# kaylode/vehicle-counting

Measured on AMD Instinct MI355X. Metric: end-to-end frames/sec (detect+NMS+ReID+track), YOLOv5s 640px, higher is better.
Workload: dtype bf16; 1 GPU; YOLOv5s 640x640 single camera stream per GPU, bf16 convs (BASELINE.json configs[1]); workload_id=s640-bf16, clip_frames=512, objects=12, num_classes=80, detection_injection=False, weights=seeded synthetic (no checkpoints available), streams=1, ranks=1, counts_allgather_via=vc_allgather_counts (RCCL, C ABI), tracked_rows=155352, tracker=device-resident (one kernel per batch, no host round trip per frame)

## Files before the change

### vehicle-counting_amd/csrc/conv_cfgs.h

```cpp
#pragma once

namespace vc {

#define VC_CONV_CFGS(X)                                                                                          \
    X(0, 256, 32, 4, 1, 4, 2)   X(1, 128, 64, 2, 2, 4, 2)   X(2, 128, 128, 2, 2, 4, 2)  X(3, 64, 64, 2, 2, 4, 2)      \
    X(4, 128, 64, 2, 2, 8, 2)   X(5, 128, 128, 2, 2, 8, 2)  X(6, 64, 64, 2, 2, 8, 2)    X(7, 256, 64, 4, 1, 4, 2)     \
    X(8, 256, 64, 4, 1, 8, 2)   X(9, 256, 128, 2, 2, 4, 2)  X(10, 256, 128, 2, 2, 8, 2) X(11, 64, 128, 1, 4, 4, 2)    \
    X(12, 64, 128, 1, 4, 8, 2)  X(13, 256, 32, 4, 1, 8, 2)                                                          \
    X(14, 64, 64, 2, 2, 4, 4)   X(15, 64, 64, 2, 2, 8, 3)   X(16, 64, 64, 2, 2, 8, 4)   X(17, 128, 64, 2, 2, 4, 4)    \
    X(18, 128, 64, 2, 2, 8, 3)  X(19, 128, 128, 2, 2, 4, 4) X(20, 128, 128, 2, 2, 8, 3) X(21, 64, 128, 1, 4, 4, 4)    \
    X(22, 64, 128, 1, 4, 8, 3)  X(23, 256, 32, 4, 1, 4, 4)  X(24, 256, 64, 4, 1, 4, 4)  X(25, 256, 64, 4, 1, 8, 3)    \
    X(26, 256, 128, 2, 2, 4, 4) X(27, 256, 128, 2, 2, 8, 3)
#define VC_HALO_CFGS(Y) Y(28, 128, 64, 2, 2, 2) Y(29, 128, 64, 2, 2, 3) Y(30, 128, 128, 2, 2, 2) Y(31, 128, 128, 2, 2, 3) \
                        Y(36, 128, 64, 4, 1, 2) Y(37, 128, 64, 4, 1, 3) Y(38, 256, 128, 4, 1, 2) Y(39, 256, 128, 4, 1, 3)
#define VC_CONV_BIG_CFGS(X) X(40, 256, 256, 4, 4, 4, 2) X(41, 256, 256, 4, 4, 4, 3) X(42, 256, 256, 4, 4, 4, 4) X(43, 256, 256, 4, 4, 8, 2)
#define VC_S2HALO_CFGS(V) V(44, 128, 128, 2, 2, 2) V(45, 128, 128, 2, 2, 3) V(46, 256, 128, 4, 1, 3) V(47, 128, 128, 2, 2, 4) \
                          V(48, 128, 256, 2, 2, 2) V(49, 256, 128, 4, 1, 2)
#define VC_DIRECT_CFGS(Z) Z(32, 2, 1, 4, 4) Z(33, 4, 2, 4, 2) Z(34, 4, 2, 2, 3) Z(35, 4, 4, 2, 2)
#define VC_STREAM_CFGS(S) S(50, 8, 4, 4, 2) S(51, 16, 8, 2, 2) S(52, 8, 8, 2, 1) S(53, 16, 4, 2, 2) S(54, 8, 4, 2, 1)
#define VC_HALO_V2_CFGS(W) W(55)
#define VC_CONV_DEEP_CFGS(X) X(60, 64, 64, 2, 2, 8, 6) X(61, 64, 64, 2, 2, 8, 8) X(62, 128, 64, 2, 2, 8, 6) X(63, 64, 128, 1, 4, 8, 6)
#define VC_SK_CFGS(K) K(56, 64, 64, 2, 2, 8, 3) K(57, 64, 64, 2, 2, 8, 4) K(58, 128, 64, 2, 2, 8, 3) K(59, 64, 128, 1, 4, 8, 3)
#define VC_PAIR_CFGS(P) P(64, 256, 128, 4, 2, 4, 3) P(65, 128, 256, 2, 4, 4, 3) P(66, 256, 128, 4, 2, 4, 2)
#define VC_PAIR4_CFGS(P) P(67, 256, 128, 2, 2, 4, 3) P(68, 256, 128, 2, 2, 4, 2)
#define VC_DIRECT8_CFGS(F) F(69, 4, 1, 2, 2) F(70, 4, 2, 2, 2) F(71, 4, 1, 4, 2) F(72, 8, 1, 2, 2)

enum ConvFamily : int { FAM_IGEMM, FAM_HALO, FAM_HALO_V2, FAM_HALO_S2, FAM_DIRECT, FAM_STREAM, FAM_DIRECT8 };
struct ConvCfgEntry { int id; ConvFamily family; };
#define VC_REG_IGEMM(i, ...) {i, FAM_IGEMM},
#define VC_REG_HALO(i, ...) {i, FAM_HALO},
#define VC_REG_HALO_V2(i, ...) {i, FAM_HALO_V2},
#define VC_REG_HALO_S2(i, ...) {i, FAM_HALO_S2},
#define VC_REG_DIRECT(i, ...) {i, FAM_DIRECT},
#define VC_REG_STREAM(i, ...) {i, FAM_STREAM},
#define VC_REG_DIRECT8(i, ...) {i, FAM_DIRECT8},
constexpr ConvCfgEntry kConvCfgs[] = {
    VC_CONV_CFGS(VC_REG_IGEMM) VC_HALO_CFGS(VC_REG_HALO) VC_DIRECT_CFGS(VC_REG_DIRECT) VC_CONV_BIG_CFGS(VC_REG_IGEMM) VC_S2HALO_CFGS(VC_REG_HALO_S2)
    VC_STREAM_CFGS(VC_REG_STREAM) VC_HALO_V2_CFGS(VC_REG_HALO_V2) VC_SK_CFGS(VC_REG_IGEMM) VC_CONV_DEEP_CFGS(VC_REG_IGEMM) VC_PAIR_CFGS(VC_REG_IGEMM)
    VC_PAIR4_CFGS(VC_REG_IGEMM) VC_DIRECT8_CFGS(VC_REG_DIRECT8)};
#undef VC_REG_IGEMM
#undef VC_REG_HALO
#undef VC_REG_HALO_V2
#undef VC_REG_HALO_S2
#undef VC_REG_DIRECT
#undef VC_REG_STREAM
#undef VC_REG_DIRECT8
constexpr int kNumConvCfgs = (int)(sizeof(kConvCfgs) / sizeof(kConvCfgs[0]));

struct ConvFamilyTable { ConvFamily of[kNumConvCfgs]; bool ok; };
constexpr ConvFamilyTable conv_family_table() {
    ConvFamilyTable t{};
    int seen[kNumConvCfgs] = {};
    t.ok = true;
    for (const ConvCfgEntry& e : kConvCfgs) {
        if (e.id < 0 || e.id >= kNumConvCfgs || seen[e.id]++) { t.ok = false; continue; }
        t.of[e.id] = e.family;
    }
    return t;
}
constexpr ConvFamilyTable kConvFamily = conv_family_table();
static_assert(kConvFamily.ok, "tile configuration ids must be exactly 0 .. N - 1, each once");

#define VC_ID_HALO_V2(i) i
constexpr int kCfgHaloV2 = VC_HALO_V2_CFGS(VC_ID_HALO_V2);
#undef VC_ID_HALO_V2

}
```

### vehicle-counting_amd/csrc/conv_dispatch.hip

```cpp
#include <algorithm>
#include <cstdlib>

#include "vc_common.h"
#include "conv_cfgs.h"

namespace vc {

int conv_num_cfgs() { return kNumConvCfgs; }

bool conv_stream_cfg(int cfg) { return cfg >= 0 && cfg < kNumConvCfgs && kConvFamily.of[cfg] == FAM_STREAM; }

int conv_k_tile(int prec) { return prec == PREC_F32 ? 32 : prec == PREC_FP8 ? 128 : 64; }

double conv_flops(const ConvP& p) { return 2.0 * (double)p.M * (double)p.Cout * (double)p.K; }

static int conv_heuristic(const ConvP& p) {
    if (p.prec == PREC_FP8) {
        if (p.Cout <= 64) return 4;
        const long t = (long)((p.M + 127) / 128) * ((p.Cout + 127) / 128);
        return t >= 512 ? 5 : 6;
    }
    if (p.in_up) return 2;
    if (p.Cout <= 32) return 0;
    if (p.Cout <= 64) return 1;
    const long t128 = (long)((p.M + 127) / 128) * ((p.Cout + 127) / 128);
    return t128 >= 512 ? 2 : 3;
}

int launch_conv_cfg(const ConvP& p, int cfg, hipStream_t s) {
    if (cfg < 0 || cfg >= conv_num_cfgs()) cfg = conv_heuristic(p);
    switch (kConvFamily.of[cfg]) {
        case FAM_IGEMM: return launch_igemm_cfg(p, cfg, s);
        case FAM_HALO: return launch_halo_cfg(p, cfg, s);
        case FAM_HALO_V2: return launch_halo_v2_cfg(p, cfg, s);
        case FAM_HALO_S2: return launch_halo_s2_cfg(p, cfg, s);
        case FAM_DIRECT:
        case FAM_STREAM:
        case FAM_DIRECT8: return launch_pointwise_cfg(p, cfg, s);
    }
    return VC_ERR_ARG;
}

int conv_check(const ConvP& p);

int launch_conv(const ConvP& p, hipStream_t s) {
    VC_TRY(conv_check(p));
    const int rc = launch_conv_cfg(p, p.cfg, s);
    if (rc == VC_ERR_ARG && p.cfg >= 0 && p.cfg < conv_num_cfgs() && !getenv("VC_CONV_STRICT")) return launch_conv_cfg(p, -1, s);
    return rc;
}

int conv_check(const ConvP& p) {
    const int ch = p.prec == PREC_F32 ? 4 : p.prec == PREC_FP8 ? 16 : 8;
    if (p.prec == PREC_FP8)
        VC_CHECK(p.scale && p.Cout % 8 == 0 && p.out_cs % 8 == 0 && p.out_co % 8 == 0 && (p.split == 0 || (p.split % 8 == 0 && p.out2_cs % 8 == 0 && p.out2_co % 8 == 0)) &&
                 (p.res_mode == RES_NONE || (p.res_cs % 4 == 0 && p.res_co % 4 == 0)), VC_ERR_ARG, "conv fp8: channel scales / 8-channel alignment of the outputs");
    VC_CHECK(p.Cin % ch == 0 && p.in_cs % ch == 0 && p.in_co % ch == 0, VC_ERR_ARG,
             "conv: input channels/stride/offset (%d,%d,%d) must be multiples of %d", p.Cin, p.in_cs, p.in_co, ch);
    VC_CHECK(p.out_cs % 4 == 0 && p.out_co % 4 == 0, VC_ERR_ARG, "conv: output stride/offset must be multiples of 4");
    VC_CHECK(p.split == 0 || (p.split % 4 == 0 && p.out2 && p.out2_cs % 4 == 0 && p.out2_co % 4 == 0 && p.res_mode == RES_NONE), VC_ERR_ARG,
             "conv: bad split destination");
    VC_CHECK(!(p.prec == PREC_FP8 && p.out_bf16 && p.split != 0), VC_ERR_ARG, "conv fp8: the bf16 store has one destination (conv_epilogue_fp8 would put channels >= split behind the first slice)");
    VC_CHECK(p.res_mode == RES_NONE || (p.res_cs % 4 == 0 && p.res_co % 4 == 0), VC_ERR_ARG, "conv: residual alignment");
    VC_CHECK(p.Kp % conv_k_tile(p.prec) == 0 && p.Kp >= p.K, VC_ERR_ARG, "conv: bad K padding %d/%d", p.K, p.Kp);
    VC_CHECK(p.M > 0 && p.Cout > 0, VC_ERR_ARG, "conv: empty problem");
    VC_CHECK(!p.in_up || (p.prec == PREC_BF16 && p.kh == 1 && p.kw == 1 && p.sh == 1 && p.sw == 1 && p.ph == 0 && p.pw == 0 && p.H % 2 == 0 && p.W % 2 == 0 &&
                          p.up_C > 0 && p.up_C < p.Cin && p.up_C % 64 == 0 && p.Cin % 64 == 0 && p.up_cs % 8 == 0 && p.up_co % 8 == 0 && !p.m_dev), VC_ERR_ARG,
             "conv: the upsample fold-in needs a bf16 pointwise conv on an even-sized map with 64-channel-aligned halves");
    VC_CHECK((size_t)p.B * p.H * p.W * p.in_cs * elem_size(p.prec) < (1ull << 31), VC_ERR_CAPACITY, "conv: input tensor exceeds the 2 GiB buffer descriptor");
    VC_CHECK((size_t)((p.Cout + 127) / 128 * 128) * p.Kp * elem_size(p.prec) < (1ull << 31), VC_ERR_CAPACITY, "conv: weights exceed 2 GiB");
    VC_CHECK(p.kh * p.kw <= 40, VC_ERR_ARG, "conv: at most 40 taps (validity mask is 64 bits incl. K padding)");
    VC_CHECK(p.M < (1 << 24), VC_ERR_CAPACITY, "conv: more than 2^24 output pixels in one launch");
    VC_CHECK((size_t)p.M * std::max(p.out_cs, std::max(p.res_cs, p.out2_cs)) * ((p.prec == PREC_F32 || p.out_f32) ? 4 : (p.prec == PREC_FP8 && !p.out_bf16) ? 1 : 2) < (1ull << 31),
             VC_ERR_CAPACITY, "conv: output tensor exceeds 2 GiB (32-bit buffer offsets)");
    return VC_OK;
}

}
```

### vehicle-counting_amd/csrc/conv_launch.h

```cpp
#pragma once
#include <algorithm>
#include <cstdint>
#include <cstdio>
#include <cstdlib>
#include <vector>

#include "vc_common.h"
#include "conv_geom.h"

namespace vc {

struct ConvSwitches {
    bool sk;
    bool s2halo;
    bool direct;
    bool direct8;
    bool halo_v2;
    bool persist;
    bool balanced;
    bool sk_uncached;
    bool s2pw_store;
    int dyn_lds;
    int reserve;
};
inline const ConvSwitches& conv_switches() {
    static const ConvSwitches sw = [] {
        const auto num = [](const char* name, int dflt) { const char* v = getenv(name); return v ? atoi(v) : dflt; };
        ConvSwitches c;
        c.sk = num("VC_CONV_SK", 1) != 0;
        c.s2halo = num("VC_CONV_S2HALO", 1) != 0;
        c.direct = num("VC_CONV_DIRECT", 1) != 0;
        c.direct8 = num("VC_CONV_DIRECT8", 1) != 0;
        c.halo_v2 = num("VC_CONV_HALO_V2", 1) != 0;
        c.persist = num("VC_CONV_PERSIST", 1) != 0;
        c.balanced = num("VC_CONV_BALANCED", 1) != 0;
        c.sk_uncached = num("VC_SK_UNCACHED", 1) != 0;
        c.s2pw_store = num("VC_S2PW_STORE", 0) != 0;
        c.dyn_lds = num("VC_CONV_DYN_LDS", 0);
        c.reserve = num("VC_CONV_RESERVE", 64);
        return c;
    }();
    return sw;
}
inline int conv_slots_reserve() { return conv_switches().reserve; }

inline int device_cus() {
    static const int n = [] {
        int dev = 0, cus = 256;
        hipDeviceProp_t prop;
        if (hipGetDevice(&dev) == hipSuccess && hipGetDeviceProperties(&prop, dev) == hipSuccess) cus = prop.multiProcessorCount;
        return cus;
    }();
    return n;
}

template <class K>
static int resident_workgroups(K kernel, int threads = 256) {
    int per_cu = 0;
    if (hipOccupancyMaxActiveBlocksPerMultiprocessor(&per_cu, kernel, threads, 0) != hipSuccess || per_cu < 1) per_cu = 1;
    return per_cu * device_cus();
}

struct WgStamps {
    const char* name;
    int n = 0, used = 0, stride = 0, w0 = 0, w1 = 0;
    long long* d = nullptr;
    size_t per_launch = 0;
    std::vector<int> grids, tiles;
    WgStamps(const char* env, const char* kernel, int max_grid, int stride_, int w0_, int w1_) : name(kernel), stride(stride_), w0(w0_), w1(w1_) {
        const char* v = getenv(env);
        n = v ? std::max(1, atoi(v)) : 0;
        per_launch = (size_t)max_grid * stride;
        if (n && hipMalloc((void**)&d, (size_t)n * per_launch * 8) != hipSuccess) { d = nullptr; n = 0; }
    }
    long long* next(int grid, int ntiles, hipStream_t s) {
        if (!d || used >= n || (size_t)grid * stride > per_launch) return nullptr;
        long long* p = d + (size_t)used++ * per_launch;
        hipMemsetAsync(p, 0, (size_t)grid * stride * 8, s);
        grids.push_back(grid); tiles.push_back(ntiles);
        return p;
    }
    template <class F>
    void report(hipStream_t s, F extra) {
        if (!d || used < n) return;
        hipStreamSynchronize(s);
        std::vector<long long> h(per_launch);
        for (int l = 0; l < used; ++l) {
            const int grid = grids[l];
            if (hipMemcpy(h.data(), d + (size_t)l * per_launch, (size_t)grid * stride * 8, hipMemcpyDeviceToHost) != hipSuccess) break;
            std::vector<double> st, du;
            long long lo = INT64_MAX, hi = 0;
            for (int b = 0; b < grid; ++b) { const long long* t = &h[(size_t)b * stride]; if (t[w0] && t[w1]) { lo = std::min(lo, t[w0]); hi = std::max(hi, t[w1]); } }
            int late = 0;
            for (int b = 0; b < grid; ++b) {
                const long long* t = &h[(size_t)b * stride];
                if (!t[w0] || !t[w1]) continue;
                st.push_back((double)(t[w0] - lo) / 100); du.push_back((double)(t[w1] - t[w0]) / 100);
                late += t[w0] - lo > 10000;
            }
            const size_t m = st.size();
            if (!m) continue;
            std::sort(st.begin(), st.end()); std::sort(du.begin(), du.end());
            fprintf(stderr, "[vc %s dbg] launch %d: %d tiles on %d workgroups; start offsets us p10/p50/p90/max %.1f %.1f %.1f %.1f ; lifetimes us p10/p50/p90/max %.1f %.1f %.1f %.1f ; "
                            "%d workgroups (%.1f %%) start > 100 us late ; first start -> last end %.1f us\n",
                    name, l, tiles[l], grid, st[m / 10], st[m / 2], st[m * 9 / 10], st[m - 1], du[m / 10], du[m / 2], du[m * 9 / 10], du[m - 1], late, 100.0 * late / m,
                    (double)(hi - lo) / 100);
            extra(h.data(), grid, tiles[l]);
        }
        used = 0; grids.clear(); tiles.clear();
    }
};

}
```

### vehicle-counting_amd/csrc/conv_pointwise.hip

```cpp
#include <algorithm>
#include <cstdlib>

#include "vc_common.h"
#include "conv_device.h"
#include "conv_cfgs.h"
#include "conv_launch.h"

namespace vc {

template <int CT, int KS, int PT, int OCC, int ACT>
__global__ __launch_bounds__(256, OCC) void conv1x1_direct_kernel(const ConvP p) {
    constexpr uint32_t OOB = 0x80000000u;
    typedef unsigned int u32x4 __attribute__((ext_vector_type(4)));
    const int lane = threadIdx.x & 63, wave = threadIdx.x >> 6;
    const int frow = lane & 15, fch = lane >> 4;
    const int NG = p.Cout / (CT * 16);
    const int gw = blockIdx.x * 4 + wave, nw = gridDim.x * 4;
    const int g = gw % NG, stride = nw / NG;
    const int nblk = (p.M + PT * 16 - 1) / (PT * 16);
    const __amdgpu_buffer_rsrc_t xsrd = __builtin_amdgcn_make_buffer_rsrc(const_cast<void*>(p.in), 0, (int)((size_t)p.B * p.H * p.W * p.in_cs * 2), 0x00020000);
    Chunk wf[CT][KS];
#pragma unroll
    for (int ct = 0; ct < CT; ++ct)
#pragma unroll
// ... 106 lines not shown

template <int CT, int KS, int PT, int NP, int ACT>
__global__ __launch_bounds__(512, 1) void conv1x1_stream_kernel(const ConvP p) {
    constexpr uint32_t OOB = 0x80000000u;
    typedef unsigned int u32x4 __attribute__((ext_vector_type(4)));
    __shared__ __attribute__((aligned(16))) uint4 wl[CT * KS * 64 + CT * 4];
    const int lane = threadIdx.x & 63, wave = threadIdx.x >> 6;
    const int frow = lane & 15, fch = lane >> 4;
    for (int f = wave; f < CT * KS; f += 8) {
        const int ks = f / CT, ct = f - ks * CT;
        wl[f * 64 + lane] = *(const uint4*)((const char*)p.w + ((size_t)(ct * 16 + frow) * p.Kw + ks * 32 + fch * 8) * 2);
    }
    float* bl = (float*)(wl + CT * KS * 64);
    for (int i = threadIdx.x; i < CT * 16; i += 512) bl[i] = p.bias[i];
    __syncthreads();
    const int gw = blockIdx.x * 8 + wave, nw = gridDim.x * 8;
    const int nblk = (p.M + PT * 16 - 1) / (PT * 16);
    const uint32_t wl_addr = (uint32_t)(uintptr_t)(__attribute__((address_space(3))) void*)wl + lane * 16;
    u32x4v x[PT][KS];
    const char* inb = (const char*)p.in + (size_t)p.in_co * 2 + fch * 16;
    const char* ra[PT];
    auto rows_of = [&](int blk) {
#pragma unroll
        for (int pt = 0; pt < PT; ++pt) ra[pt] = inb + (size_t)min((blk * PT + pt) * 16 + frow, p.M - 1) * p.in_cs * 2;
    };
#define VC_XLOAD(pt, ks) asm volatile("global_load_dwordx4 %0, %1, off offset:%2" : "=v"(x[pt][ks]) : "v"(ra[pt]), "n"((ks) * 64))
    rows_of(gw);
#pragma unroll
    for (int ks = 0; ks < KS; ++ks)
#pragma unroll
        for (int pt = 0; pt < PT; ++pt) VC_XLOAD(pt, ks);
    constexpr int CTP = CT / NP;
    for (int blk = gw; blk < nblk; blk += nw) {
        rows_of(blk + nw);
#pragma unroll
        for (int np = 0; np < NP; ++np) {
            f32x4 acc[CTP][PT];
#pragma unroll
            for (int a = 0; a < CTP; ++a)
#pragma unroll
                for (int b = 0; b < PT; ++b) acc[a][b] = (f32x4){0.f, 0.f, 0.f, 0.f};
            uint32_t wa = wl_addr + np * CTP * 1024;
            asm volatile("" : "+v"(wa));
            u32x4v wcur, wnext;
            asm volatile("ds_read_b128 %0, %1" : "=v"(wcur) : "v"(wa));
#pragma unroll
            for (int ks = 0; ks < KS; ++ks) {
                if (np == 0) {
                    asm volatile("s_waitcnt vmcnt(%0)" ::"n"((KS - 1 - ks) * PT));
#pragma unroll
                    for (int b = 0; b < PT; ++b) asm volatile("" : "+v"(x[b][ks]));
                }
#pragma unroll
                for (int a = 0; a < CTP; ++a) {
                    if (a + 1 < CTP) asm volatile("ds_read_b128 %0, %1 offset:%2" : "=v"(wnext) : "v"(wa), "n"((a + 1) * 1024));
                    else if (ks + 1 < KS) { wa += CT * 1024; asm volatile("ds_read_b128 %0, %1" : "=v"(wnext) : "v"(wa)); }
                    if (a + 1 < CTP || ks + 1 < KS) asm volatile("s_waitcnt lgkmcnt(1)" : "+v"(wcur));
                    else asm volatile("s_waitcnt lgkmcnt(0)" : "+v"(wcur));
                    Chunk wf;
                    wf.u = wcur;
#pragma unroll
                    for (int b = 0; b < PT; ++b) {
                        Chunk xa;
                        xa.u = x[b][ks];
                        acc[a][b] = __builtin_amdgcn_mfma_f32_16x16x32_bf16(wf.h, xa.h, acc[a][b], 0, 0, 0);
                    }
                    wcur = wnext;
                }
                if (np == NP - 1) {
#pragma unroll
                    for (int b = 0; b < PT; ++b) VC_XLOAD(b, ks);
                }
            }
#pragma unroll
            for (int a = 0; a < CTP; ++a) {
                const float4 b1[1] = {*(const float4*)(bl + (np * CTP + a) * 16 + fch * 4)};
                conv_epilogue_bf16<PT, 1, ACT, RES_NONE>(p, reinterpret_cast<f32x4(&)[1][PT]>(acc[a]), b1, blk * PT * 16, (np * CTP + a) * 16 + fch * 4, frow);
            }
        }
    }
}
#undef VC_XLOAD

static bool direct1x1_applicable(const ConvP& p, int ct, int ks) {
    if (p.prec != PREC_BF16 || p.kh != 1 || p.kw != 1 || p.sh != 1 || p.sw != 1 || p.ph != 0 || p.pw != 0) return false;
    if (p.Cin != ks * 32 || p.K != p.Cin || p.Ho != p.H || p.Wo != p.W || p.in_cs % 8 != 0 || p.in_co % 8 != 0 || p.in_up || p.m_dev) return false;
    if (p.out_f32 || p.res_mode != RES_NONE || (p.act != ACT_SILU && p.act != ACT_NONE) || p.out_cs % 8 != 0 || p.out_co % 8 != 0) return false;
    if (p.split != 0 && (p.split % 8 != 0 || p.out2_cs % 8 != 0 || p.out2_co % 8 != 0)) return false;
    const int ng = p.Cout / (ct * 16);
    return p.Cout % (ct * 16) == 0 && (ng == 1 || ng == 2 || ng == 4);
}

template <int CT, int KS, int PT, int OCC>
static int launch_direct1x1(ConvP p, hipStream_t s) {
    if (!conv_switches().direct || !direct1x1_applicable(p, CT, KS)) return VC_ERR_ARG;
    p.Kw = p.Kp;
    const int ng = p.Cout / (CT * 16);
    const int nblk = (p.M + PT * 16 - 1) / (PT * 16);
    const int need = (nblk * ng + 3) / 4;
    static const int slots_hw = resident_workgroups(conv1x1_direct_kernel<CT, KS, PT, OCC, ACT_SILU>);
    const int slots = p.slots > 0 ? p.slots : std::max(256, slots_hw - conv_slots_reserve());
    p.ntiles = nblk * ng;
    if (p.act == ACT_SILU) launch_timed(p, conv1x1_direct_kernel<CT, KS, PT, OCC, ACT_SILU>, dim3(std::min(need, slots)), dim3(256), 0, s, p);
    else launch_timed(p, conv1x1_direct_kernel<CT, KS, PT, OCC, ACT_NONE>, dim3(std::min(need, slots)), dim3(256), 0, s, p);
    VC_HIP(hipGetLastError());
    return VC_OK;
}

static bool direct8_applicable(const ConvP& p, int ct, int ks) {
    if (p.prec != PREC_FP8 || p.kh != 1 || p.kw != 1 || p.sh != 1 || p.sw != 1 || p.ph != 0 || p.pw != 0) return false;
    if (p.K != p.Cin || p.Cin > ks * 128 || p.Cin <= (ks - 1) * 128 || p.Cin % 64 != 0 || (p.Cin % 128 != 0 && p.Cin != 64)) return false;
    if (p.Ho != p.H || p.Wo != p.W || p.in_cs % 16 != 0 || p.in_co % 16 != 0 || p.in_up || p.m_dev || !p.scale || p.Kw < ks * 128) return false;
    const int ng = (p.Cout + ct * 16 - 1) / (ct * 16);
    return ng == 1 || ng == 2 || ng == 4;
}

template <int CT, int KS, int PT, int OCC>
static int launch_direct8(ConvP p, hipStream_t s) {
    p.Kw = p.Kp;
    if (!conv_switches().direct8 || !direct8_applicable(p, CT, KS)) return VC_ERR_ARG;
    const int ng = (p.Cout + CT * 16 - 1) / (CT * 16);
    const int nblk = (p.M + PT * 16 - 1) / (PT * 16);
    const int need = (nblk * ng + 3) / 4;
    static const int slots_hw = resident_workgroups(conv1x1_direct_fp8_kernel<CT, KS, PT, OCC>);
    const int slots = p.slots > 0 ? p.slots : std::max(256, slots_hw - conv_slots_reserve());
    p.ntiles = nblk * ng;
    launch_timed(p, conv1x1_direct_fp8_kernel<CT, KS, PT, OCC>, dim3(std::min(need, slots)), dim3(256), 0, s, p);
    VC_HIP(hipGetLastError());
    return VC_OK;
}

template <int CT, int KS, int PT, int NP>
static int launch_stream1x1(ConvP p, hipStream_t s) {
    if (!direct1x1_applicable(p, CT, KS) || p.Cout != CT * 16) return VC_ERR_ARG;
    p.Kw = p.Kp;
    const int nblk = (p.M + PT * 16 - 1) / (PT * 16);
    p.ntiles = nblk;
    const int grid = std::max(1, std::min((nblk + 7) / 8, p.slots > 0 ? std::max(1, p.slots / 8) : device_cus()));
    if (p.act == ACT_SILU) launch_timed(p, conv1x1_stream_kernel<CT, KS, PT, NP, ACT_SILU>, dim3(grid), dim3(512), 0, s, p);
    else launch_timed(p, conv1x1_stream_kernel<CT, KS, PT, NP, ACT_NONE>, dim3(grid), dim3(512), 0, s, p);
    VC_HIP(hipGetLastError());
    return VC_OK;
}

int launch_pointwise_cfg(const ConvP& p, int cfg, hipStream_t s) {
    switch (cfg) {
#define VC_Z(i, ct, ks, pt, occ) case i: return launch_direct1x1<ct, ks, pt, occ>(p, s);
        VC_DIRECT_CFGS(VC_Z)
#undef VC_Z
#define VC_S(i, ct, ks, pt, np) case i: return launch_stream1x1<ct, ks, pt, np>(p, s);
        VC_STREAM_CFGS(VC_S)
#undef VC_S
#define VC_F(i, ct, ks, pt, occ) case i: return launch_direct8<ct, ks, pt, occ>(p, s);
        VC_DIRECT8_CFGS(VC_F)
#undef VC_F
    }
    return VC_ERR_ARG;
}

}
```

### vehicle-counting_amd/csrc/engine_run.hip

```cpp
#include <algorithm>
#include <cmath>
#include <cstdlib>

#include "engine.h"

namespace vc {

static std::string tune_key(const ConvP& c) {
    int bucket = 1;
    while (bucket < c.M) bucket <<= 1;
    char k[160];
    snprintf(k, sizeof(k), "p%d_ci%d_co%d_k%dx%d_s%d_h%d_w%d_K%d_m%d_sp%d%s", c.prec, c.Cin, c.Cout, c.kh, c.kw, c.sh, c.H, c.W, c.K, bucket, c.split,
             c.in_up ? "_up" : "");
    return k;
}

static std::mutex g_tune_mu;
static std::map<std::string, int> g_tuned;

void tune_cache_load(vc_engine* e) {
    const char* path = getenv("VC_TUNE_CACHE");
    if (!path) return;
    FILE* f = fopen(path, "r");
    if (!f) return;
    char k[200];
    int cfg;
    while (fscanf(f, "%199s %d", k, &cfg) == 2) e->tuned[k] = cfg;
    fclose(f);
}

void tune_cache_save(vc_engine* e) {
    const char* path = getenv("VC_TUNE_CACHE");
    if (!path || !e->tuned_dirty) return;
    FILE* f = fopen(path, "w");
    if (!f) return;
    for (const auto& kv : e->tuned) fprintf(f, "%s %d\n", kv.first.c_str(), kv.second);
    fclose(f);
}

void tune_cache_publish(vc_engine* e) {
    std::lock_guard<std::mutex> lk(g_tune_mu);
    for (const auto& kv : e->tuned) g_tuned["d" + std::to_string(e->cfg.device) + "_" + kv.first] = kv.second;
}

void plans_retune(vc_engine* e) {
    for (auto& kv : e->yolo_plans) for (Op& op : kv.second.ops) op.tuned = -2;
    for (auto& kv : e->reid_plans) for (Op& op : kv.second.ops) op.tuned = -2;
}

static int tuned_cfg(vc_engine* e, const ConvP& c, hipStream_t s) {
    static const bool enabled = !(getenv("VC_AUTOTUNE") && atoi(getenv("VC_AUTOTUNE")) == 0);
    if (!enabled) return -1;
    const std::string key = tune_key(c);
    auto it = e->tuned.find(key);
    if (it != e->tuned.end()) return it->second;
    const std::string gkey = "d" + std::to_string(e->cfg.device) + "_" + key;
    {
        std::lock_guard<std::mutex> lk(g_tune_mu);
        auto g = g_tuned.find(gkey);
        if (g != g_tuned.end()) { e->tuned[key] = g->second; e->tuned_dirty = true; return g->second; }
    }
    int best = -1;
    float best_ms = 1e30f;
    static const bool stream_on = getenv("VC_CONV_STREAM") && atoi(getenv("VC_CONV_STREAM")) != 0;
    for (int cfg = 0; cfg < conv_num_cfgs(); ++cfg) {
        if (conv_stream_cfg(cfg) && !stream_on) continue;
        if (launch_conv_cfg(c, cfg, s) != VC_OK) continue;
        float tmin = 1e30f;
        for (int rep = 0; rep < 3; ++rep) {
            hipEventRecord(e->ev0, s);
            launch_conv_cfg(c, cfg, s);
            hipEventRecord(e->ev1, s);
            hipEventSynchronize(e->ev1);
            float ms = 0.f;
            hipEventElapsedTime(&ms, e->ev0, e->ev1);
            tmin = std::min(tmin, ms);
        }
        static const bool tlog = getenv("VC_TUNE_LOG") != nullptr;
        if (tlog) fprintf(stderr, "[vc tune] %s cfg %d %.4f ms\n", key.c_str(), cfg, tmin);
        if (tmin < best_ms) { best_ms = tmin; best = cfg; }
    }
    e->tuned[key] = best;
    e->tuned_dirty = true;
    {
        std::lock_guard<std::mutex> lk(g_tune_mu);
        g_tuned.emplace(gkey, best);
    }
    return best;
}

static void conv_timer_arm(vc_engine* e, ConvP& cp, double flops, double bytes, const Op& op) {
    if (!e->prof_async || e->profiling || e->prof_used >= e->prof_pairs.size()) return;
    vc_engine::ProfPair& pp = e->prof_pairs[e->prof_used++];
    pp.flops = flops; pp.bytes = bytes;
    pp.rows = op.rows_level >= 0 && e->h_hc_ring ? e->h_hc_ring + (size_t)e->hc_ring_cur * 4 + op.rows_level : nullptr;
    pp.flops_per_row = op.flops_per_row; pp.bytes_per_row = op.bytes_per_row;
    pp.flops_dense = op.dense_flops >= 0 ? op.dense_flops : -1; pp.bytes_dense = op.dense_bytes >= 0 ? op.dense_bytes : -1;
    cp.ev_start = pp.a; cp.ev_stop = pp.b;
}

struct ConvCtx {
    vc_engine* e;
    ConvP& cp;
    Op* op; size_t left;
    hipStream_t s;
    bool u8_src = false;
    const View* q8 = nullptr;
};
struct ConvLaunch {
    int (*launch)(ConvCtx&);
    int n_ops;
    int cfg;
    double flops, bytes;
    int N, K, kh, kw, sh;
};
static double conv_flops(const Op& o) { return 2.0 * o.conv.M * (double)o.conv.Cout * o.C; }

static int conv_select(ConvCtx& c, double fl, double by, ConvLaunch& L) {
    vc_engine* e = c.e;
    ConvP& cp = c.cp;
    Op& op = *c.op;
    const double es = elem_size(cp.prec);
    auto conv_at = [&](size_t j) -> const Op* { return j < c.left && c.op[j].kind == Op::CONV ? &c.op[j] : nullptr; };
    const Op *nx = c.left > 1 ? &c.op[1] : nullptr, *o1 = conv_at(1), *o2 = conv_at(2), *o3 = conv_at(3);
    const double in_bytes = (double)cp.B * cp.H * cp.W * cp.Cin * es;
    auto w_bytes = [&](const Op& o) { return (double)o.conv.Cout * o.conv.K * es; };
    auto out_bytes = [&](const Op& o) { return (double)o.conv.M * o.conv.Cout * es; };
    L = {nullptr, 1, -1, fl, by, op.conv.Cout, op.conv.K, op.conv.kh, op.conv.kw, op.conv.sh};
    auto fused = [&](int cfg, int n_ops, double flops, double bytes, int N, int K, int k, int sh) {
        L.cfg = cfg; L.n_ops = n_ops; L.flops = flops; L.bytes = bytes; L.N = N; L.K = K; L.kh = L.kw = k; L.sh = sh;
    };

    const bool front_ok = e->opt.front_fused > 0 && o1 && front_fused_applicable(cp, o1->conv);
    c.u8_src = e->stem_src && cp.in == e->ybuf["in"].ptr;
    const bool stem_ok = e->opt.stem_direct != 0 && stem_direct_applicable(cp);
// ... 311 lines not shown
```

### vehicle-counting_amd/csrc/vc_common.h

```cpp
#pragma once
#include <hip/hip_runtime.h>
#include <hip/hip_ext.h>
#include <cmath>
#include <cstdint>
#include <cstdio>
#include <cstring>
#include <string>

#include "../../include/vcount_hip.h"

namespace vc {

void set_error(const char* fmt, ...);
const char* last_error();

#define VC_HIP(expr)                                                                            \
    do {                                                                                        \
        hipError_t _e = (expr);                                                                 \
        if (_e != hipSuccess) {                                                                 \
            vc::set_error("%s:%d %s -> %s", __FILE__, __LINE__, #expr, hipGetErrorString(_e));  \
            return VC_ERR_HIP;                                                                  \
        }                                                                                       \
    } while (0)

// ... 79 lines not shown
        s0 = s; s1 = s + 1 < src - 1 ? s + 1 : src - 1;
    } else {
        s0 = s < 0 ? 0 : (s > src - 1 ? src - 1 : s);
        s1 = s + 1 < 0 ? 0 : (s + 1 > src - 1 ? src - 1 : s + 1);
    }
    const float w0 = (1.f - f) * 2048.f, w1 = f * 2048.f;
#if defined(__HIP_DEVICE_COMPILE__)
    int r0 = __float2int_rn(w0), r1 = __float2int_rn(w1);
#else
    int r0 = (int)nearbyintf(w0), r1 = (int)nearbyintf(w1);
#endif
    c0 = r0 < -32768 ? -32768 : (r0 > 32767 ? 32767 : r0);
    c1 = r1 < -32768 ? -32768 : (r1 > 32767 ? 32767 : r1);
}

enum Act : int { ACT_NONE = 0, ACT_SILU = 1, ACT_RELU = 2 };
enum ResMode : int { RES_NONE = 0, RES_AFTER_ACT = 1, RES_BEFORE_ACT = 2 };

struct ConvP {
    const void* in;
    const void* w;
    const float* bias;
    const void* res;
    void* out;
    int B, H, W, Cin;
    int in_cs, in_co;
    int Ho, Wo, Cout;
    int out_cs, out_co;
    int res_cs, res_co;
    int kh, kw, sh, sw, ph, pw;
    int K, Kp;
    int Kw;
    int act, res_mode, out_f32, prec;
    const float* scale;
    float act_scale, inv_act_scale;
    int out_bf16;
    int M;
    int cfg;
    hipEvent_t ev_start, ev_stop;
    int ntiles;
    void* out2;
    int split, out2_cs, out2_co;
    const int* m_dev;
    const void* in_up;
    int up_C, up_cs, up_co;
    int ksplit;
    float* sk_ws;
    int* sk_tickets;
    long long* dbg;
    int s2_th, s2_tw;
    int slots;
    int ablate;
    unsigned* tile_ctr;
};

#if defined(__HIPCC__)
__device__ __forceinline__ int tile_claim(unsigned* ctr) {
    return (int)gridDim.x + (int)__hip_atomic_fetch_add(ctr, 1u, __ATOMIC_RELAXED, __HIP_MEMORY_SCOPE_AGENT);
}
__device__ __forceinline__ int tile_claim_chunk(unsigned* ctr) {
    return (int)__hip_atomic_fetch_add(ctr, 1u, __ATOMIC_RELAXED, __HIP_MEMORY_SCOPE_AGENT);
}
__device__ __forceinline__ void tile_claims_done(unsigned* ctr) {
    if (__hip_atomic_fetch_add(ctr + 1, 1u, __ATOMIC_RELAXED, __HIP_MEMORY_SCOPE_AGENT) == gridDim.x - 1) {
        __hip_atomic_store(ctr, 0u, __ATOMIC_RELAXED, __HIP_MEMORY_SCOPE_AGENT);
        __hip_atomic_store(ctr + 1, 0u, __ATOMIC_RELAXED, __HIP_MEMORY_SCOPE_AGENT);
    }
}
#endif

template <class K, class... A>
static inline void launch_timed(const ConvP& p, K kernel, dim3 grid, dim3 block, unsigned lds, hipStream_t s, A... args) {
    if (p.ev_start) hipExtLaunchKernelGGL(kernel, grid, block, lds, s, p.ev_start, p.ev_stop, 0, args...);
    else hipLaunchKernelGGL(kernel, grid, block, lds, s, args...);
}

int launch_conv(const ConvP& p, hipStream_t s);
int launch_conv_cfg(const ConvP& p, int cfg, hipStream_t s);
int launch_igemm_cfg(const ConvP& p, int cfg, hipStream_t s);
int launch_halo_cfg(const ConvP& p, int cfg, hipStream_t s);
int launch_halo_v2_cfg(const ConvP& p, int cfg, hipStream_t s);
int launch_halo_s2_cfg(const ConvP& p, int cfg, hipStream_t s);
int launch_pointwise_cfg(const ConvP& p, int cfg, hipStream_t s);
bool s2halo_pw_applicable(const ConvP& p, const ConvP& q);
int launch_s2halo_pw(ConvP p, ConvP q, hipStream_t s);
int conv_num_cfgs();
bool conv_stream_cfg(int cfg);
bool stem_direct_applicable(const ConvP& p);
struct View;
int launch_stem_direct(const ConvP& p, hipStream_t s, const View* q8 = nullptr, float q_inv_scale = 1.0f, int grid_cap = 0);
struct LetterboxGeom;
bool stem_u8_applicable(const ConvP& p, const LetterboxGeom& g);
int launch_stem_direct_u8(const ConvP& p, const uint8_t* frames, const LetterboxGeom& g, hipStream_t s, const View* q8 = nullptr, float q_inv_scale = 1.0f, int grid_cap = 0);
bool c3_fused_applicable(const ConvP& p12, const ConvP& pm1, const ConvP& pm2, const ConvP& p3);
int launch_c3_fused(const ConvP& p12, const ConvP& pm1, const ConvP& pm2, const ConvP& p3, hipStream_t s, int grid_cap = 0);
bool bneck_fused_applicable(const ConvP& pm1, const ConvP& pm2);
int launch_bneck_fused(const ConvP& pm1, const ConvP& pm2, hipStream_t s, int grid_cap = 0);
bool bneck_cv3_fused_applicable(const ConvP& pm1, const ConvP& pm2, const ConvP& p3);
int launch_bneck_cv3_fused(const ConvP& pm1, const ConvP& pm2, const ConvP& p3, hipStream_t s, int grid_cap = 0);
bool front_fused_applicable(const ConvP& p0, const ConvP& p1);
int launch_front_fused(const ConvP& p0, const ConvP& p1, const uint8_t* frames_u8 , const LetterboxGeom& g, hipStream_t s);
bool front_fused_resize_ok(const LetterboxGeom& g);
bool reid_block_fused_applicable(const ConvP& p1, const ConvP& p2);
int launch_reid_block_fused(const ConvP& p1, const ConvP& p2, hipStream_t s, int grid_cap = 0);
bool reid_stem_applicable(const ConvP& p, int out_cs, int out_co);
int launch_reid_stem_pool(const ConvP& p, void* pooled, hipStream_t s);
int conv_k_tile(int prec);
double conv_flops(const ConvP& p);

}
```

Before: 24070 frames/s.

## Add weight-register-resident 1x1 conv kernel family to autotuner candidates

Adds a new persistent 1x1 bf16 convolution kernel that keeps the whole weight slice in registers and streams activation tiles through a multi-stage LDS ring using buffer-to-LDS loads. It also overlaps each tile's epilogue with the next tile's MFMA work. The configs are registered as a new family the autotuner can pick, plus an env override to force them. The aim is to cut repeated weight loads and hide memory latency for pointwise convs, at the cost of high register pressure and only being used where the tuner selects it.

Result: faster. 25040 frames/s (median of 6 runs) (+4.0%).

```diff
diff --git a/vehicle-counting_amd/csrc/conv_cfgs.h b/vehicle-counting_amd/csrc/conv_cfgs.h
--- a/vehicle-counting_amd/csrc/conv_cfgs.h
+++ b/vehicle-counting_amd/csrc/conv_cfgs.h
@@ -24,8 +24,9 @@
 #define VC_PAIR_CFGS(P) P(64, 256, 128, 4, 2, 4, 3) P(65, 128, 256, 2, 4, 4, 3) P(66, 256, 128, 4, 2, 4, 2)
 #define VC_PAIR4_CFGS(P) P(67, 256, 128, 2, 2, 4, 3) P(68, 256, 128, 2, 2, 4, 2)
 #define VC_DIRECT8_CFGS(F) F(69, 4, 1, 2, 2) F(70, 4, 2, 2, 2) F(71, 4, 1, 4, 2) F(72, 8, 1, 2, 2)
+#define VC_WREG_CFGS(W) W(73, 8, 4, 2, 3) W(74, 8, 4, 2, 4) W(75, 8, 2, 2, 2) W(76, 4, 4, 2, 4) W(77, 4, 2, 2, 3) W(78, 4, 2, 2, 4)
 
-enum ConvFamily : int { FAM_IGEMM, FAM_HALO, FAM_HALO_V2, FAM_HALO_S2, FAM_DIRECT, FAM_STREAM, FAM_DIRECT8 };
+enum ConvFamily : int { FAM_IGEMM, FAM_HALO, FAM_HALO_V2, FAM_HALO_S2, FAM_DIRECT, FAM_STREAM, FAM_DIRECT8, FAM_WREG };
 struct ConvCfgEntry { int id; ConvFamily family; };
 #define VC_REG_IGEMM(i, ...) {i, FAM_IGEMM},
 #define VC_REG_HALO(i, ...) {i, FAM_HALO},
@@ -34,10 +35,11 @@
 #define VC_REG_DIRECT(i, ...) {i, FAM_DIRECT},
 #define VC_REG_STREAM(i, ...) {i, FAM_STREAM},
 #define VC_REG_DIRECT8(i, ...) {i, FAM_DIRECT8},
+#define VC_REG_WREG(i, ...) {i, FAM_WREG},
 constexpr ConvCfgEntry kConvCfgs[] = {
     VC_CONV_CFGS(VC_REG_IGEMM) VC_HALO_CFGS(VC_REG_HALO) VC_DIRECT_CFGS(VC_REG_DIRECT) VC_CONV_BIG_CFGS(VC_REG_IGEMM) VC_S2HALO_CFGS(VC_REG_HALO_S2)
     VC_STREAM_CFGS(VC_REG_STREAM) VC_HALO_V2_CFGS(VC_REG_HALO_V2) VC_SK_CFGS(VC_REG_IGEMM) VC_CONV_DEEP_CFGS(VC_REG_IGEMM) VC_PAIR_CFGS(VC_REG_IGEMM)
-    VC_PAIR4_CFGS(VC_REG_IGEMM) VC_DIRECT8_CFGS(VC_REG_DIRECT8)};
+    VC_PAIR4_CFGS(VC_REG_IGEMM) VC_DIRECT8_CFGS(VC_REG_DIRECT8) VC_WREG_CFGS(VC_REG_WREG)};
 #undef VC_REG_IGEMM
 #undef VC_REG_HALO
 #undef VC_REG_HALO_V2
@@ -45,6 +47,7 @@
 #undef VC_REG_DIRECT
 #undef VC_REG_STREAM
 #undef VC_REG_DIRECT8
+#undef VC_REG_WREG
 constexpr int kNumConvCfgs = (int)(sizeof(kConvCfgs) / sizeof(kConvCfgs[0]));
 
 struct ConvFamilyTable { ConvFamily of[kNumConvCfgs]; bool ok; };
diff --git a/vehicle-counting_amd/csrc/conv_dispatch.hip b/vehicle-counting_amd/csrc/conv_dispatch.hip
--- a/vehicle-counting_amd/csrc/conv_dispatch.hip
+++ b/vehicle-counting_amd/csrc/conv_dispatch.hip
@@ -37,6 +37,7 @@
         case FAM_DIRECT:
         case FAM_STREAM:
         case FAM_DIRECT8: return launch_pointwise_cfg(p, cfg, s);
+        case FAM_WREG: return launch_wreg_cfg(p, cfg, s);
     }
     return VC_ERR_ARG;
 }
diff --git a/vehicle-counting_amd/csrc/conv_launch.h b/vehicle-counting_amd/csrc/conv_launch.h
--- a/vehicle-counting_amd/csrc/conv_launch.h
+++ b/vehicle-counting_amd/csrc/conv_launch.h
@@ -15,6 +15,7 @@
     bool s2halo;
     bool direct;
     bool direct8;
+    bool wreg;
     bool halo_v2;
     bool persist;
     bool balanced;
@@ -31,6 +32,7 @@
         c.s2halo = num("VC_CONV_S2HALO", 1) != 0;
         c.direct = num("VC_CONV_DIRECT", 1) != 0;
         c.direct8 = num("VC_CONV_DIRECT8", 1) != 0;
+        c.wreg = num("VC_CONV_WREG", 1) != 0;
         c.halo_v2 = num("VC_CONV_HALO_V2", 1) != 0;
         c.persist = num("VC_CONV_PERSIST", 1) != 0;
         c.balanced = num("VC_CONV_BALANCED", 1) != 0;
diff --git a/vehicle-counting_amd/csrc/conv_pointwise.hip b/vehicle-counting_amd/csrc/conv_pointwise.hip
--- a/vehicle-counting_amd/csrc/conv_pointwise.hip
+++ b/vehicle-counting_amd/csrc/conv_pointwise.hip
@@ -212,6 +212,139 @@
 }
 #undef VC_XLOAD
 
+template <int KS, int NG, int PT, int NS, int ACT>
+__global__ __launch_bounds__(256, 2) void conv1x1_wreg_kernel(const ConvP p) {
+    constexpr int CT = 4;
+    constexpr int NPP = 4 / NG;
+    constexpr int BP = PT * 16 * NPP;
+    constexpr int KCH = KS * 4;
+    constexpr int RPI = 64 / KCH;
+    constexpr int XI = BP * KS / 64;
+    constexpr int STAGE = BP * KCH;
+    constexpr int NGRP = (PT / 2) * CT;
+    static_assert(NG == 2 || NG == 4, "channel groups per workgroup");
+    static_assert(KS == 4 || KS == 8, "K = 128 or 256");
+    static_assert(PT % 2 == 0 && (BP * KS) % 64 == 0 && XI >= 1 && PT * 16 * KCH * 16 + 256 < 65536, "tile shape");
+    static_assert(NS >= 2 && NS * STAGE * 16 <= 64 * 1024, "the ring: at most 64 KB, two workgroups and a neighbour per CU");
+    static_assert((NS - 2) * XI + (NS - 1) * 2 * NGRP <= 63, "the counted s_waitcnt must fit vmcnt");
+    __shared__ __attribute__((aligned(256))) uint4 lds[NS * STAGE];
+    typedef __attribute__((address_space(3))) void* lds_ptr_t;
+    if (p.ablate == 6) return;
+
+    const int lane = threadIdx.x & 63, wave = threadIdx.x >> 6;
+    const int uwave = __builtin_amdgcn_readfirstlane(wave);
+    const int frow = lane & 15, fch = lane >> 4;
+    const int g = uwave % NG, pp = uwave / NG;
+    const int ntiles = p.ntiles, G = gridDim.x;
+    const __amdgpu_buffer_rsrc_t xsrd = __builtin_amdgcn_make_buffer_rsrc(const_cast<void*>(p.in), 0, (int)((size_t)p.B * p.H * p.W * p.in_cs * 2), 0x00020000);
+
+    const int srow = wave * RPI + lane / KCH;
+    const uint32_t soff0 = (uint32_t)((srow * p.in_cs + p.in_co) * 2 + ((lane % KCH) ^ (srow & 15)) * 16);
+    const uint32_t soff1 = RPI == 2 ? (uint32_t)((srow * p.in_cs + p.in_co) * 2 + ((lane % KCH) ^ ((srow & 15) ^ 8)) * 16) : soff0;
+    const uint32_t row_bytes = (uint32_t)(p.in_cs * 2);
+    int s_v = blockIdx.x, s_buf = 0, s_issued = 0;
+    auto stage_next = [&]() {
+        if (!((p.ablate == 1 || p.ablate == 3) && s_issued >= NS)) {
+            const int m0 = s_v < ntiles ? s_v * BP : p.M;
+#pragma unroll
+            for (int i = 0; i < XI; ++i) {
+                const uint32_t o = (uint32_t)(m0 + i * 4 * RPI) * row_bytes + ((RPI == 2 && (i & 1)) ? soff1 : soff0);
+                __builtin_amdgcn_raw_ptr_buffer_load_lds(xsrd, (lds_ptr_t)&lds[s_buf * STAGE + (i * 4 + uwave) * 64], 16, (int)o, 0, 0, 0);
+            }
+        }
+        ++s_issued;
+        s_v += G;
+        s_buf = s_buf + 1 == NS ? 0 : s_buf + 1;
+        asm volatile("" ::: "memory");
+    };
+#pragma unroll
+    for (int st = 0; st < NS - 1; ++st) stage_next();
+
+    Chunk wf[CT][KS];
+#pragma unroll
+    for (int ct = 0; ct < CT; ++ct)
+#pragma unroll
+        for (int ks = 0; ks < KS; ++ks)
+            wf[ct][ks].u = *(const u32x4v*)((const char*)p.w + ((size_t)((g * CT + ct) * 16 + frow) * p.Kw + ks * 32 + fch * 8) * 2);
+    float bias_l = p.bias[g * 64 + lane];
+#pragma unroll
+    for (int ct = 0; ct < CT; ++ct)
+#pragma unroll
+        for (int ks = 0; ks < KS; ++ks) asm volatile("" : "+v"(wf[ct][ks].u));
+    asm volatile("" : "+v"(bias_l));
+
+    uint32_t xa = (uint32_t)(uintptr_t)(lds_ptr_t)&lds[0] + (uint32_t)((pp * PT * 16 + frow) * (KCH * 16) + (fch ^ (frow & 3)) * 16 + (frow >> 2) * 64);
+    constexpr uint32_t STAGE_BYTES = STAGE * 16;
+    int rbuf = 0;
+
+    f32x4 acc[CT][PT], prev[CT][PT];
+#pragma unroll
+    for (int a = 0; a < CT; ++a)
+#pragma unroll
+        for (int b = 0; b < PT; ++b) prev[a][b] = (f32x4){0.f, 0.f, 0.f, 0.f};
+    int prev_m = p.M;
+    const int nbase = g * CT * 16 + fch * 4;
+    auto epilogue_group = [&](int gi) {
+        const int b = gi / CT * 2, a = gi % CT;
+        float bv[4];
+        int bsel = fch * 16;
+        asm volatile("" : "+v"(bsel));
+#pragma unroll
+        for (int j = 0; j < 4; ++j) bv[j] = __int_as_float(__builtin_amdgcn_ds_bpermute(bsel + (a * 16 + j) * 4, __float_as_int(bias_l)));
+        const float4 b1[1] = {make_float4(bv[0], bv[1], bv[2], bv[3])};
+        conv_epilogue_bf16<2, 1, ACT, RES_NONE>(p, reinterpret_cast<f32x4(&)[1][2]>(prev[a][b]), b1, prev_m + b * 16, nbase + a * 16, frow);
+    };
+#define VC_XREAD(dst, f)                                                                                                   \
+    asm volatile("ds_read_b128 %0, %1 offset:%2" : "=v"(dst) : "v"(xa ^ (uint32_t)((((f) / PT) & 3) * 64)), "n"(((f) % PT) * 16 * KCH * 16 + (((f) / PT) >> 2) * 256) : "memory")
+
+    asm volatile("s_waitcnt vmcnt(%0)" ::"n"((NS - 2) * XI) : "memory");
+    __builtin_amdgcn_s_barrier();
+    for (int v = blockIdx.x; v < ntiles; v += G) {
+        stage_next();
+#pragma unroll
+        for (int a = 0; a < CT; ++a)
+#pragma unroll
+            for (int b = 0; b < PT; ++b) acc[a][b] = (f32x4){0.f, 0.f, 0.f, 0.f};
+        u32x4v x[2];
+        VC_XREAD(x[0], 0);
+#pragma unroll
+        for (int f = 0; f < KS * PT; ++f) {
+            if (f + 1 < KS * PT) {
+                VC_XREAD(x[(f + 1) & 1], f + 1);
+                asm volatile("s_waitcnt lgkmcnt(1)" ::: "memory");
+            } else {
+                asm volatile("s_waitcnt lgkmcnt(0)" ::: "memory");
+            }
+            asm volatile("" : "+v"(x[f & 1]));
+            Chunk xf;
+            xf.u = x[f & 1];
+#pragma unroll
+            for (int a = 0; a < CT; ++a) acc[a][f % PT] = __builtin_amdgcn_mfma_f32_16x16x32_bf16(wf[a][f / PT].h, xf.h, acc[a][f % PT], 0, 0, 0);
+            if (f % PT == PT - 1) {
+#pragma unroll
+                for (int gi = (f / PT) * NGRP / KS; gi < (f / PT + 1) * NGRP / KS; ++gi) epilogue_group(gi);
+            }
+        }
+#pragma unroll
+        for (int a = 0; a < CT; ++a)
+#pragma unroll
+            for (int b = 0; b < PT; ++b) prev[a][b] = acc[a][b];
+        prev_m = v * BP + pp * PT * 16;
+        {
+            const uint32_t step = rbuf + 1 == NS ? 0u - (NS - 1) * STAGE_BYTES : STAGE_BYTES;
+            rbuf = rbuf + 1 == NS ? 0 : rbuf + 1;
+            xa += step;
+        }
+        if (p.split == 0) asm volatile("s_waitcnt vmcnt(%0)" ::"n"((NS - 2) * XI + (NS - 1) * NGRP) : "memory");
+        else asm volatile("s_waitcnt vmcnt(%0)" ::"n"((NS - 2) * XI + (NS - 1) * 2 * NGRP) : "memory");
+        __builtin_amdgcn_s_barrier();
+    }
+#undef VC_XREAD
+#pragma unroll
+    for (int gi = 0; gi < NGRP; ++gi) epilogue_group(gi);
+    asm volatile("s_waitcnt vmcnt(0)" ::: "memory");
+}
+
 static bool direct1x1_applicable(const ConvP& p, int ct, int ks) {
     if (p.prec != PREC_BF16 || p.kh != 1 || p.kw != 1 || p.sh != 1 || p.sw != 1 || p.ph != 0 || p.pw != 0) return false;
     if (p.Cin != ks * 32 || p.K != p.Cin || p.Ho != p.H || p.Wo != p.W || p.in_cs % 8 != 0 || p.in_co % 8 != 0 || p.in_up || p.m_dev) return false;
@@ -271,6 +404,46 @@
     else launch_timed(p, conv1x1_stream_kernel<CT, KS, PT, NP, ACT_NONE>, dim3(grid), dim3(512), 0, s, p);
     VC_HIP(hipGetLastError());
     return VC_OK;
+}
+
+bool wreg_applicable(const ConvP& p, int ks, int ng) {
+    if (p.prec != PREC_BF16 || p.kh != 1 || p.kw != 1 || p.sh != 1 || p.sw != 1 || p.ph != 0 || p.pw != 0) return false;
+    if (p.Cin != ks * 32 || p.K != p.Cin || p.Cout != ng * 64 || p.Ho != p.H || p.Wo != p.W || p.in_up || p.m_dev) return false;
+    if (p.in_cs % 8 != 0 || p.in_co % 8 != 0 || p.out_cs % 8 != 0 || p.out_co % 8 != 0) return false;
+    if (p.out_f32 || p.res_mode != RES_NONE || (p.act != ACT_SILU && p.act != ACT_RELU && p.act != ACT_NONE)) return false;
+    return p.split == 0 || (p.split % 8 == 0 && p.out2_cs % 8 == 0 && p.out2_co % 8 == 0);
+}
+
+template <int KS, int NG, int PT, int NS>
+static int launch_wreg(ConvP p, hipStream_t s) {
+    const ConvSwitches& sw = conv_switches();
+    if (!sw.wreg || !wreg_applicable(p, KS, NG)) return VC_ERR_ARG;
+    constexpr int BP = PT * 16 * (4 / NG);
+    p.Kw = p.Kp;
+    p.ntiles = (p.M + BP - 1) / BP;
+    static const int slots_hw = resident_workgroups(conv1x1_wreg_kernel<KS, NG, PT, NS, ACT_SILU>);
+    const int grid = p.slots > 0 ? std::min(p.ntiles, p.slots) : persistent_grid(p.ntiles, slots_hw, sw.reserve, 0, sw.balanced);
+    if (p.act == ACT_SILU) launch_timed(p, conv1x1_wreg_kernel<KS, NG, PT, NS, ACT_SILU>, dim3(grid), dim3(256), 0, s, p);
+    else if (p.act == ACT_RELU) launch_timed(p, conv1x1_wreg_kernel<KS, NG, PT, NS, ACT_RELU>, dim3(grid), dim3(256), 0, s, p);
+    else launch_timed(p, conv1x1_wreg_kernel<KS, NG, PT, NS, ACT_NONE>, dim3(grid), dim3(256), 0, s, p);
+    VC_HIP(hipGetLastError());
+    return VC_OK;
+}
+
+int wreg_cfg_for(const ConvP& p) {
+#define VC_W(i, ks, ng, pt, ns) if (wreg_applicable(p, ks, ng)) return i;
+    VC_WREG_CFGS(VC_W)
+#undef VC_W
+    return -1;
+}
+
+int launch_wreg_cfg(const ConvP& p, int cfg, hipStream_t s) {
+    switch (cfg) {
+#define VC_W(i, ks, ng, pt, ns) case i: return launch_wreg<ks, ng, pt, ns>(p, s);
+        VC_WREG_CFGS(VC_W)
+#undef VC_W
+    }
+    return VC_ERR_ARG;
 }
 
 int launch_pointwise_cfg(const ConvP& p, int cfg, hipStream_t s) {
diff --git a/vehicle-counting_amd/csrc/engine_run.hip b/vehicle-counting_amd/csrc/engine_run.hip
--- a/vehicle-counting_amd/csrc/engine_run.hip
+++ b/vehicle-counting_amd/csrc/engine_run.hip
@@ -51,6 +51,7 @@
 static int tuned_cfg(vc_engine* e, const ConvP& c, hipStream_t s) {
     static const bool enabled = !(getenv("VC_AUTOTUNE") && atoi(getenv("VC_AUTOTUNE")) == 0);
     if (!enabled) return -1;
+    if (const char* fw = getenv("VC_TUNE_WREG")) return atoi(fw) != 0 ? wreg_cfg_for(c) : -1;
     const std::string key = tune_key(c);
     auto it = e->tuned.find(key);
     if (it != e->tuned.end()) return it->second;
diff --git a/vehicle-counting_amd/csrc/vc_common.h b/vehicle-counting_amd/csrc/vc_common.h
--- a/vehicle-counting_amd/csrc/vc_common.h
+++ b/vehicle-counting_amd/csrc/vc_common.h
@@ -185,6 +185,9 @@
 int launch_halo_v2_cfg(const ConvP& p, int cfg, hipStream_t s);
 int launch_halo_s2_cfg(const ConvP& p, int cfg, hipStream_t s);
 int launch_pointwise_cfg(const ConvP& p, int cfg, hipStream_t s);
+int launch_wreg_cfg(const ConvP& p, int cfg, hipStream_t s);
+bool wreg_applicable(const ConvP& p, int ks, int ng);
+int wreg_cfg_for(const ConvP& p);
 bool s2halo_pw_applicable(const ConvP& p, const ConvP& q);
 int launch_s2halo_pw(ConvP p, ConvP q, hipStream_t s);
 int conv_num_cfgs();
```
